# rodluger/starry_process

Measured on AMD Instinct MI355X. Metric: log_likelihood evals/sec (ydeg=15, K=1000), higher is better.
Workload: dtype f64

## Files before the change

### starry_process_amd/csrc/sp_cov.h

```cpp
#ifndef SP_COV_H
#define SP_COV_H

#include "sp_internal.h"

__device__ __forceinline__ int star_nobs(const sp_star &st, int K) {
  return (st.nobs > 0 && st.nobs < K) ? st.nobs : K;
}

__device__ __forceinline__ double temporal_factor(int kind, double ti, double tj,
                                                  double tau) {
#pragma clang fp contract(off)
  if (kind == SP_TEMPORAL_NONE) return 1.0;
  const double dt = fabs(ti - tj);
  if (kind == SP_TEMPORAL_MATERN32) {
    const double x = 1.7320508075688772 * dt / tau;
    return (1.0 + x) * exp(-x);
  }
  return exp(-(dt * dt) / (2.0 * tau));
}

__device__ __forceinline__ double temporal_dfactor_dtau(int kind, double ti, double tj,
                                                        double tau) {
  if (kind == SP_TEMPORAL_NONE) return 0.0;
  const double dt = fabs(ti - tj);
  if (kind == SP_TEMPORAL_MATERN32) {
    const double x = 1.7320508075688772 * dt / tau;
    return x * x / tau * exp(-x);
  }
  return (dt * dt) / (2.0 * tau * tau) * exp(-(dt * dt) / (2.0 * tau));
}

template <int CTRL>
__device__ __forceinline__ double dpp_move(double v) {
  const int lo = __builtin_amdgcn_mov_dpp(__double2loint(v), CTRL, 0xf, 0xf, true);
  const int hi = __builtin_amdgcn_mov_dpp(__double2hiint(v), CTRL, 0xf, 0xf, true);
  return __hiloint2double(hi, lo);
}
template <int N>
__device__ __forceinline__ void row16_sum(double (&x)[N]) {
#pragma unroll
  for (int k = 0; k < N; ++k) x[k] += dpp_move<0xB1>(x[k]);
#pragma unroll
  for (int k = 0; k < N; ++k) x[k] += dpp_move<0x4E>(x[k]);
#pragma unroll
  for (int k = 0; k < N; ++k) x[k] += dpp_move<0x141>(x[k]);
#pragma unroll
  for (int k = 0; k < N; ++k) x[k] += dpp_move<0x140>(x[k]);
}

typedef double dd2 __attribute__((ext_vector_type(2)));

struct SplineGen {
  const double *tab;
  int np2;
  double dx, inv_dx;
  int covpts;
  __device__ __forceinline__ double operator()(double thi, double thj) const {
#pragma clang fp contract(off)
    const double x = fabs(thi - thj);
    const double q = x * inv_dx;
    int idx = (int)q;
    double x0 = q - (double)idx;
    if (fabs(x0 - 0.5) > 0.5 - 1.0e-9) {
      idx = (int)floor(x / dx);
      x0 = q - (double)idx;
    }
    idx = idx > covpts ? covpts : idx;
    typedef const __attribute__((address_space(3))) dd2 *lds_dd2;
    const unsigned a1 = (unsigned)(size_t)(const __attribute__((address_space(3))) double *)tab + ((unsigned)idx << 4);
    const dd2 c01 = *(lds_dd2)(size_t)a1;
    const dd2 c23 = *(lds_dd2)(size_t)(a1 + 8u * (unsigned)np2);
    return __builtin_fma(x0, __builtin_fma(x0, __builtin_fma(x0, c23.y, c23.x), c01.y), c01.x);
  }
  template <int N>
  __device__ __forceinline__ void many(const double (&thi)[N], const double (&thj)[N], double (&out)[N]) const {
#pragma clang fp contract(off)
    double x0[N];
    int idx[N];
    bool odd = false;
#pragma unroll
    for (int e = 0; e < N; ++e) {
      const double q = fabs(thi[e] - thj[e]) * inv_dx;
      idx[e] = (int)q;
      x0[e] = q - (double)idx[e];
      odd |= fabs(x0[e] - 0.5) > 0.5 - 1.0e-9;
    }
    if (__builtin_expect(odd, 0)) {
#pragma unroll
      for (int e = 0; e < N; ++e)
        if (fabs(x0[e] - 0.5) > 0.5 - 1.0e-9) {
          const double x = fabs(thi[e] - thj[e]);
          idx[e] = (int)floor(x / dx);
          x0[e] = x * inv_dx - (double)idx[e];
        }
    }
    dd2 c01[N], c23[N];
    typedef const __attribute__((address_space(3))) dd2 *lds_dd2;
    const unsigned base = (unsigned)(size_t)(const __attribute__((address_space(3))) double *)tab;
    const unsigned off2 = 8u * (unsigned)np2;
#pragma unroll
    for (int e = 0; e < N; ++e) {
      const int k = idx[e] > covpts ? covpts : idx[e];
      const unsigned a1 = base + ((unsigned)k << 4);
      c01[e] = *(lds_dd2)(size_t)a1;
      c23[e] = *(lds_dd2)(size_t)(a1 + off2);
    }
#pragma unroll
    for (int e = 0; e < N; ++e)
      out[e] = __builtin_fma(x0[e], __builtin_fma(x0[e], __builtin_fma(x0[e], c23[e].y, c23[e].x), c01[e].y), c01[e].x);
  }
};


__device__ __forceinline__ void spline_table_to_lds(const double *__restrict__ src, double *stage, int np, int tid) {
  const int n2 = 2 * np;
  dd2 v[4];
#pragma unroll
  for (int c = 0; c < 4; ++c) {
    const int e = tid + 256 * c;
    v[c] = e < n2 ? *reinterpret_cast<const dd2 *>(src + 2 * e) : dd2{0.0, 0.0};
  }
#pragma unroll
  for (int c = 0; c < 4; ++c) {
    const int e = tid + 256 * c;
    if (e < n2) *reinterpret_cast<dd2 *>(stage + 2 * e) = v[c];
  }
  for (int e = tid + 1024; e < n2; e += 256)
    *reinterpret_cast<dd2 *>(stage + 2 * e) = *reinterpret_cast<const dd2 *>(src + 2 * e);
}


#ifndef SP_LAZY_BATCH
#define SP_LAZY_BATCH 8
#endif
template <int MA, typename V4>
__device__ __forceinline__ void lazy_cov_tiles(const LazyCov &z, int star, const int (&ri)[MA][4],
                                               const int (&cj)[4], V4 (&out)[MA][4], double *stage) {
  const sp_star st = z.stars[star];
  const int nobs = star_nobs(st, z.K), np = z.covpts + 4;
  const double *th = z.theta + (size_t)star * z.K, *tt = z.t + (size_t)star * z.K;
  const bool tk = z.temporal != SP_TEMPORAL_NONE;
#ifdef SP_LAZY_NO_SEP
  const bool sep = false;
#else
  const bool sep = z.temporal == SP_TEMPORAL_MATERN32 && z.inorder && z.inorder[star] != 0.0;
#endif
  double thi[MA][4], ti[MA][4], thj[4], tj[4];
#pragma unroll
  for (int k = 0; k < 4; ++k) {
    const bool oj = cj[k] < nobs;
    thj[k] = oj ? th[cj[k]] : 0.0;
    tj[k] = (oj && tk) ? tt[cj[k]] : 0.0;
#pragma unroll
    for (int m = 0; m < MA; ++m) {
      const bool oi = ri[m][k] < nobs;
      thi[m][k] = oi ? th[ri[m][k]] : 0.0;
      ti[m][k] = (oi && tk) ? tt[ri[m][k]] : 0.0;
    }
  }
  const int c0 = cj[0] & ~63;
  const double tb = sep ? tt[c0 < nobs ? c0 : nobs - 1] : 0.0;
  spline_table_to_lds(z.ptab + (size_t)star * 4 * np, stage, np, threadIdx.x);
  __syncthreads();
  SplineGen g{stage, 2 * np, 6.283185307179586 / z.covpts,
              1.0 / (6.283185307179586 / z.covpts), z.covpts};
  const double cm = sep ? 1.7320508075688772 / st.tau : 0.0;
  double fc[4] = {1.0, 1.0, 1.0, 1.0};
  bool fok[4] = {false, false, false, false};
  if (sep) {
#pragma unroll
    for (int n = 0; n < 4; ++n) {
      const double a = cm * (tj[n] - tb);
      fok[n] = a < 600.0 && a >= 0.0;
      fc[n] = exp(fok[n] ? a : 0.0);
    }
  }
#pragma unroll
  for (int m = 0; m < MA; ++m) {
    double er[4] = {1.0, 1.0, 1.0, 1.0};
    if (sep) {
#pragma unroll
      for (int r = 0; r < 4; ++r) er[r] = exp(-(cm * (ti[m][r] - tb)));
    }
#pragma unroll
    for (int n0 = 0; n0 < 4; n0 += SP_LAZY_BATCH / 4) {
      double a[SP_LAZY_BATCH], b[SP_LAZY_BATCH], v[SP_LAZY_BATCH];
#pragma unroll
      for (int e = 0; e < SP_LAZY_BATCH; ++e) {
        a[e] = thi[m][e & 3];
        b[e] = thj[n0 + (e >> 2)];
      }
      g.many<SP_LAZY_BATCH>(a, b, v);
#pragma unroll
      for (int e = 0; e < SP_LAZY_BATCH; ++e) {
        const int n = n0 + (e >> 2), r = e & 3;
        double w = 0.0;
        if (ri[m][r] < nobs && cj[n] < nobs) {
#pragma clang fp contract(off)
          if (sep && fok[n]) {
            const double x = cm * (ti[m][r] - tj[n]);
            w = v[e] * ((1.0 + x) * (er[r] * fc[n]));
          } else {
            w = v[e] * temporal_factor(z.temporal, ti[m][r], tj[n], st.tau);
          }
        }
        out[m][n][r] = w;
      }
    }
    if (z.rid) {
#pragma unroll
      for (int r = 0; r < 4; ++r) {
        const int mr = ri[m][r] - z.K;
        if (mr < 0 || mr >= z.nrid) continue;
        const double *src = z.rid + ((size_t)star * (z.nrid + 1) + mr) * z.K;
        double x[4];
#pragma unroll
        for (int n = 0; n < 4; ++n) x[n] = src[cj[n] < z.K ? cj[n] : z.K - 1];
#pragma unroll
        for (int n = 0; n < 4; ++n) out[m][n][r] = cj[n] < z.K ? x[n] : 0.0;
      }
    }
  }
  __syncthreads();
}

template <typename V4>
__device__ __forceinline__ void lazy_diag_block(const LazyCov &z, int star, const SplineGen &g, const sp_star &st,
                                                int nobs, const int (&ri)[4], int cj, V4 &out) {
  const double *th = z.theta + (size_t)star * z.K, *tt = z.t + (size_t)star * z.K;
  const double *rb = z.rid + (size_t)star * (z.nrid + 1) * z.K;
  const bool tk = z.temporal != SP_TEMPORAL_NONE;
  const int cc = cj < z.K ? cj : z.K - 1;
  const double thj = th[cc], tj = tk ? tt[cc] : 0.0;
  double thi[4], ti[4], dd[4], rv[4];
#pragma unroll
  for (int r = 0; r < 4; ++r) {
    const int rc = ri[r] < z.K ? ri[r] : z.K - 1;
    thi[r] = th[rc];
    ti[r] = tk ? tt[rc] : 0.0;
    dd[r] = rb[(size_t)z.nrid * z.K + rc];
    const int m = ri[r] - z.K;
    rv[r] = rb[(size_t)((m >= 0 && m < z.nrid) ? m : 0) * z.K + cc];
  }
#pragma unroll
  for (int r = 0; r < 4; ++r) {
    const int m = ri[r] - z.K;
    double v;
    if (ri[r] < nobs && cj < nobs) {
#pragma clang fp contract(off)
      v = g(thi[r], thj) * temporal_factor(z.temporal, ti[r], tj, st.tau);
      if (ri[r] == cj) v += dd[r];
    } else if (m >= 0 && m < z.nrid && cj < z.K) {
      v = rv[r];
    } else {
      v = ri[r] == cj ? 1.0 : 0.0;
    }
    out[r] = v;
  }
}

#ifndef SP_LAZY_ROW_BATCH
#define SP_LAZY_ROW_BATCH 0
#endif
template <int ROWB, typename V4>
__device__ __forceinline__ void lazy_cov_row(const LazyCov &z, int star, int ri, int c0, V4 (&out)[4],
                                             double *stage, int tid) {
  const sp_star st = z.stars[star];
  const int nobs = star_nobs(st, z.K), np = z.covpts + 4;
  const double *th = z.theta + (size_t)star * z.K;
  const bool oi = ri < nobs;
  const double thi = oi ? th[ri] : 0.0;
  double *s_thj = stage + 4 * np;
  {
    const double *src = z.ptab + (size_t)star * 4 * np;
    const int n2 = 2 * np, cbase = c0 & ~63;
    dd2 v[3];
#pragma unroll
    for (int c = 0; c < 3; ++c) {
      const int e = tid + 256 * c;
      v[c] = e < n2 ? *reinterpret_cast<const dd2 *>(src + 2 * e) : dd2{0.0, 0.0};
    }
    const double tj = (tid < 64 && cbase + tid < nobs) ? th[cbase + tid] : 0.0;
#pragma unroll
    for (int c = 0; c < 3; ++c) {
      const int e = tid + 256 * c;
      if (e < n2) *reinterpret_cast<dd2 *>(stage + 2 * e) = v[c];
    }
    for (int e = tid + 768; e < n2; e += 256)
      *reinterpret_cast<dd2 *>(stage + 2 * e) = *reinterpret_cast<const dd2 *>(src + 2 * e);
    if (tid < 64) s_thj[tid] = tj;
  }
  __syncthreads();
  SplineGen g{stage, 2 * np, 6.283185307179586 / z.covpts,
              1.0 / (6.283185307179586 / z.covpts), z.covpts};
  const int cl = c0 & 63;
  if constexpr (ROWB == 2) {
#pragma unroll
  for (int m = 0; m < 4; ++m) {
    V4 o;
#pragma unroll
    for (int half = 0; half < 2; ++half) {
      const dd2 tt = *reinterpret_cast<const dd2 *>(s_thj + cl + 16 * m + 2 * half);
      const double a[2] = {thi, thi}, b[2] = {tt.x, tt.y};
      double v[2];
      g.many<2>(a, b, v);
      o[2 * half] = (oi && c0 + 16 * m + 2 * half < nobs) ? v[0] : 0.0;
      o[2 * half + 1] = (oi && c0 + 16 * m + 2 * half + 1 < nobs) ? v[1] : 0.0;
      __builtin_amdgcn_sched_barrier(0);
    }
    out[m] = o;
  }
  } else if constexpr (ROWB == 0) {
#pragma unroll
  for (int m = 0; m < 4; ++m) {
    const dd2 t01 = *reinterpret_cast<const dd2 *>(s_thj + cl + 16 * m), t23 = *reinterpret_cast<const dd2 *>(s_thj + cl + 16 * m + 2);
    const double thj[4] = {t01.x, t01.y, t23.x, t23.y};
    V4 o;
#pragma unroll
    for (int r = 0; r < 4; ++r) o[r] = (oi && c0 + 16 * m + r < nobs) ? g(thi, thj[r]) : 0.0;
    out[m] = o;
  }
  } else {
#pragma unroll
  for (int m0 = 0; m0 < 4; m0 += ROWB / 4) {
    double a[ROWB], b[ROWB], v[ROWB];
#pragma unroll
    for (int h = 0; h < ROWB / 4; ++h) {
      const dd2 t01 = *reinterpret_cast<const dd2 *>(s_thj + cl + 16 * (m0 + h));
      const dd2 t23 = *reinterpret_cast<const dd2 *>(s_thj + cl + 16 * (m0 + h) + 2);
      a[4 * h] = a[4 * h + 1] = a[4 * h + 2] = a[4 * h + 3] = thi;
      b[4 * h] = t01.x;
      b[4 * h + 1] = t01.y;
      b[4 * h + 2] = t23.x;
      b[4 * h + 3] = t23.y;
    }
    g.many<ROWB>(a, b, v);
#pragma unroll
    for (int h = 0; h < ROWB / 4; ++h) {
      V4 o;
#pragma unroll
      for (int r = 0; r < 4; ++r) o[r] = (oi && c0 + 16 * (m0 + h) + r < nobs) ? v[4 * h + r] : 0.0;
      out[m0 + h] = o;
    }
    __builtin_amdgcn_sched_barrier(0);
  }
  }
  if (z.rid && !oi) {
    const int mr = ri - z.K;
    if (mr >= 0 && mr < z.nrid) {
      const double *src = z.rid + ((size_t)star * (z.nrid + 1) + mr) * z.K;
      double x[16];
#pragma unroll
      for (int e = 0; e < 16; ++e) {
        const int c = c0 + 16 * (e >> 2) + (e & 3);
        x[e] = src[c < z.K ? c : z.K - 1];
      }
#pragma unroll
      for (int m = 0; m < 4; ++m) {
        V4 o;
#pragma unroll
        for (int r = 0; r < 4; ++r) o[r] = c0 + 16 * m + r < z.K ? x[4 * m + r] : 0.0;
        out[m] = o;
      }
    }
  }
  __syncthreads();
}

#endif
```

### starry_process_amd/csrc/sp_gemm.hip

```cpp
#include <cstdlib>

#include <type_traits>

#include "sp_internal.h"
#include "sp_tile.h"
#include "sp_cov.h"
#include "sp_mm.h"
#include "sp_stage.h"
#include "sp_paneldiag.h"

typedef double d2 __attribute__((ext_vector_type(2)));

#define GT SP_GT

namespace {

__global__ __launch_bounds__(256) void gemm_nt_kernel(
    const double *A, long lda, long strideA, const double *__restrict__ B, long ldb, long strideB,
    double *C, long ldc, long strideC, int Mrows, int Nrows, int Kd, double alpha, int beta,
    int lower_only, int batch, int ntn, int ntiles, const int32_t *__restrict__ bsel, int nsel) {
  constexpr int BK = 32, LDW = BK + 1;
  __shared__ __attribute__((aligned(16))) double smem[2 * GT * LDW];
  double *sA = smem, *sB = smem + GT * LDW;
  int mtx, tile;
  if (!sp_xcd_decode(blockIdx.x, batch, ntiles, mtx, tile)) return;
  int ti, tj;
  if (lower_only) {
    ti = (int)((sqrt(8.0 * tile + 1.0) - 1.0) * 0.5);
    while (ti * (ti + 1) / 2 > tile) --ti;
    while ((ti + 1) * (ti + 2) / 2 <= tile) ++ti;
    tj = tile - ti * (ti + 1) / 2;
  } else {
    ti = tile / ntn;
    tj = tile % ntn;
  }
  const int row0 = ti * GT, col0 = tj * GT;
  const double *Ab = A + (size_t)mtx * strideA;
  int bm = mtx;
  if (bsel) {
    bm = bsel[mtx];
    if (bm < 0 || bm >= nsel) bm = 0;
  }
  const double *Bb = B + (size_t)bm * strideB;
  double *Cb = C + (size_t)mtx * strideC;
  const int lane = threadIdx.x & 63, wave = threadIdx.x >> 6;
  const int fr = lane & 15, fk = lane >> 4;
  d4 acc[4];
#pragma unroll
  for (int n = 0; n < 4; ++n) acc[n] = d4{0.0, 0.0, 0.0, 0.0};
  const bool full = row0 + GT <= Mrows && col0 + GT <= Nrows;
  if (beta) {
#pragma unroll
    for (int n = 0; n < 4; ++n)
#pragma unroll
      for (int r = 0; r < 4; ++r) {
        const int gi = row0 + 16 * wave + fk + 4 * r, gj = col0 + 16 * n + fr;
        if (full || (gi < Mrows && gj < Nrows)) acc[n][r] = Cb[(size_t)gi * ldc + gj];
      }
  }
  const bool vecA = ((lda & 1) == 0) && ((reinterpret_cast<uintptr_t>(Ab) & 15) == 0);
  const bool vecB = ((ldb & 1) == 0) && ((reinterpret_cast<uintptr_t>(Bb) & 15) == 0);
  PanelRegs<BK> ra, rb;
  if (Kd > 0) {
    stage_load<BK>(Ab, lda, row0, Mrows, 0, Kd, vecA, ra);
    stage_load<BK>(Bb, ldb, col0, Nrows, 0, Kd, vecB, rb);
  }
  for (int k0 = 0; k0 < Kd; k0 += BK) {
    stage_store<BK>(ra, alpha, sA);
    stage_store<BK>(rb, 1.0, sB);
    __syncthreads();
    if (k0 + BK < Kd) {
      stage_load<BK>(Ab, lda, row0, Mrows, k0 + BK, Kd, vecA, ra);
      stage_load<BK>(Bb, ldb, col0, Nrows, k0 + BK, Kd, vecB, rb);
    }
    const double *pa = sA + (16 * wave + fr) * LDW + fk;
    const double *pb = sB + fr * LDW + fk;
#pragma unroll
    for (int kk = 0; kk < BK; kk += 4) {
      const double a = pa[kk];
      acc[0] = __builtin_amdgcn_mfma_f64_16x16x4f64(a, pb[kk], acc[0], 0, 0, 0);
      acc[1] = __builtin_amdgcn_mfma_f64_16x16x4f64(a, pb[16 * LDW + kk], acc[1], 0, 0, 0);
      acc[2] = __builtin_amdgcn_mfma_f64_16x16x4f64(a, pb[32 * LDW + kk], acc[2], 0, 0, 0);
      acc[3] = __builtin_amdgcn_mfma_f64_16x16x4f64(a, pb[48 * LDW + kk], acc[3], 0, 0, 0);
    }
    __syncthreads();
  }
#pragma unroll
  for (int n = 0; n < 4; ++n)
#pragma unroll
    for (int r = 0; r < 4; ++r) {
      const int gi = row0 + 16 * wave + fk + 4 * r, gj = col0 + 16 * n + fr;
      if (full || (gi < Mrows && gj < Nrows)) Cb[(size_t)gi * ldc + gj] = acc[n][r];
    }
}

}

namespace {
#ifdef SP_MM_STAMPS
__device__ long long sp_mm_dbg[8 * 4096];
#endif
#ifndef SP_MM_WAVES
#define SP_MM_WAVES 1
#endif
#ifndef SP_MM_SYRK_NS
#define SP_MM_SYRK_NS 6
#endif
template <class Core, bool SGN, bool SEL = false>
__global__ __launch_bounds__(256, SP_MM_WAVES) void mm_nt_kernel(
    const double *__restrict__ A, long lda, long strideA, const double *__restrict__ B, long ldb,
    long strideB, double *__restrict__ C, long ldc, long strideC, int Kd, double alpha, int beta,
    int lower_only, int batch, int ntn, int ntiles, int skip00, LazyCov lz, DiagFuse df,
    const int32_t *__restrict__ bsel, int nsel) {
  constexpr int TM = Core::TM_, TN = Core::TN_;
  static_assert(Core::LDS_DOUBLES >= SP_DIAG_LDS_DOUBLES, "the tile-(0,0) workgroup factors a pivot block in this LDS");
  __shared__ __attribute__((aligned(16))) double lds[Core::LDS_DOUBLES];
#ifdef SP_MM_STAMPS
  const long long wall_begin = wall_clock64(), cyc_begin = __builtin_readcyclecounter();
#endif
  int mtx, tile;
  if (!sp_xcd_decode(blockIdx.x, batch, ntiles, mtx, tile)) return;
  int ti, tj;
  if (lower_only) {
    ti = (int)((sqrt(8.0 * tile + 1.0) - 1.0) * 0.5);
    while (ti * (ti + 1) / 2 > tile) --ti;
    while ((ti + 1) * (ti + 2) / 2 <= tile) ++ti;
    tj = tile - ti * (ti + 1) / 2;
  } else {
    ti = tile / ntn;
    tj = tile % ntn;
  }
  const int tj_limit = skip00 >> 8;
  int k_first = (skip00 & 2) ? ti * TM : 0;
  if (df.tri0 >= 0 && TM == 64) {
    const int r = 64 * (df.j + ti) - df.tri0, first = r > 0 ? r / 64 - df.s0 : 0;
    if (first > 0) k_first = 64 * first < Kd ? 64 * first : Kd;
  }
  if (tj_limit && tj >= tj_limit) return;
  if ((skip00 & 1) && lower_only && ti == 0 && tj == 0) {
    if (df.sys) {
      __builtin_amdgcn_s_setprio(3);
      panel_diag_item(df.sys + (size_t)mtx * df.stride, df.ld, df.j, df.nact,
                      df.img + (size_t)mtx * df.lts + sp_img_off(df.j),
                      df.info ? df.info + mtx : nullptr, lds, threadIdx.x);
    }
    return;
  }
  const double *Ab = A + (size_t)mtx * strideA + (size_t)ti * TM * lda;
  int bm = mtx;
  if constexpr (SEL) {
    bm = bsel[mtx];
    if (bm < 0 || bm >= nsel) bm = 0;
  }
  const double *Bb = B + (size_t)bm * strideB + (size_t)tj * TN * ldb;
  double *Cb = C + (size_t)mtx * strideC + (size_t)ti * TM * ldc + (size_t)tj * TN;
  Core mm;
  mm.init(Ab, lda, Bb, ldb);
  if constexpr (SGN && Core::MA == 1 && Core::NA == 4 && TM == 64 && TN == 64) {
    if ((skip00 & 4) && lower_only && ti == tj) {
      const bool dform = beta && lz.theta && (lz.dlazy & 2);
      const int lane = threadIdx.x & 63;
      sp_star dst{};
      int dnobs = 0;
      if (dform) {
        dst = lz.stars[mtx];
        dnobs = star_nobs(dst, lz.K);
        spline_table_to_lds(lz.ptab + (size_t)mtx * 4 * (lz.covpts + 4), lds, lz.covpts + 4, threadIdx.x);
        __syncthreads();
      }
      const SplineGen dg{lds, 2 * (lz.covpts + 4), 6.283185307179586 / lz.covpts, 1.0 / (6.283185307179586 / lz.covpts),
                         lz.covpts};
      if (!dform) mm.prologue(lds, k_first, Kd);
      auto run = [&](auto wtag) {
        constexpr int W = decltype(wtag)::value;
        using D = typename Core::template SymDeal<W>;
        mm_d4 a3[3];
#pragma unroll
        for (int b = 0; b < 3; ++b) {
          mm_d4 c = mm_d4{0.0, 0.0, 0.0, 0.0};
          if (b < D::NB && dform) {
            int ri[4];
#pragma unroll
            for (int r = 0; r < 4; ++r) ri[r] = 64 * (lz.tr0 + ti) + 16 * D::brow(b) + (lane >> 4) + 4 * r;
            lazy_diag_block(lz, mtx, dg, dst, dnobs, ri, 64 * (lz.tc0 + tj) + 16 * D::bcol(b) + (lane & 15), c);
          } else if (b < D::NB && beta) {
#pragma unroll
            for (int r = 0; r < 4; ++r)
              c[r] = Cb[(size_t)(16 * D::brow(b) + (lane >> 4) + 4 * r) * ldc + 16 * D::bcol(b) + (lane & 15)];
          }
          a3[b] = alpha < 0.0 ? -c : c;
        }
        if (dform) {
          __syncthreads();
          mm.prologue(lds, k_first, Kd);
        }
        mm.template sym_loop<W>(lds, k_first, Kd, a3);
#pragma unroll
        for (int b = 0; b < D::NB; ++b)
#pragma unroll
          for (int r = 0; r < 4; ++r)
            Cb[(size_t)(16 * D::brow(b) + (lane >> 4) + 4 * r) * ldc + 16 * D::bcol(b) + (lane & 15)] =
                alpha < 0.0 ? -a3[b][r] : a3[b][r];
      };
      switch (threadIdx.x >> 6) {
        case 0: run(std::integral_constant<int, 0>{}); break;
        case 1: run(std::integral_constant<int, 1>{}); break;
        case 2: run(std::integral_constant<int, 2>{}); break;
        default: run(std::integral_constant<int, 3>{}); break;
      }
      return;
    }
  }
  mm_d4 acc[Core::MA][Core::NA], cin[SGN ? 1 : Core::MA][SGN ? 1 : Core::NA];
  constexpr bool CAN_LAZY = Core::MA == 1 && Core::NA == 4 && TM == 64 && TN == 64;
  const bool lazy = CAN_LAZY && beta && lz.theta && lz.tr0 + ti > lz.tc0 + tj && lz.tc0 + tj > 0 &&
                    lz.tr0 + ti < lz.nfull;
  mm_d4 cz1[1][4];
  mm_d4 (&cz)[4] = cz1[0];
  if (!lazy) mm.prologue(lds, k_first, Kd);
  if (lazy) {
    int ri[1][4], cj[4];
#pragma unroll
    for (int k = 0; k < 4; ++k) {
      ri[0][k] = 64 * (lz.tr0 + ti) + mm.acc_row(0, k);
      cj[k] = 64 * (lz.tc0 + tj) + mm.acc_col(k < Core::NA ? k : 0);
    }
    lazy_cov_tiles<1>(lz, mtx, ri, cj, cz1, lds);
    mm.prologue(lds, k_first, Kd);
  }
#pragma unroll
  for (int m = 0; m < Core::MA; ++m)
#pragma unroll
    for (int n = 0; n < Core::NA; ++n) {
      mm_d4 c = mm_d4{0.0, 0.0, 0.0, 0.0};
      if (lazy) {
        c = cz[n & 3];
      } else if (beta) {
#pragma unroll
        for (int r = 0; r < 4; ++r) c[r] = Cb[(size_t)mm.acc_row(m, r) * ldc + mm.acc_col(n)];
      }
      if (SGN) {
        acc[m][n] = alpha < 0.0 ? -c : c;
      } else {
        acc[m][n] = mm_d4{0.0, 0.0, 0.0, 0.0};
        cin[m][n] = c;
      }
    }
#ifdef SP_MM_STAMPS
  const long long cyc_loop = __builtin_readcyclecounter();
#endif
  mm.loop(lds, k_first, Kd, acc);
#ifdef SP_MM_STAMPS
  const long long cyc_store = __builtin_readcyclecounter();
#endif
#pragma unroll
  for (int m = 0; m < Core::MA; ++m)
#pragma unroll
    for (int n = 0; n < Core::NA; ++n)
#pragma unroll
      for (int r = 0; r < 4; ++r) {
        double v;
        if (SGN)
          v = alpha < 0.0 ? -acc[m][n][r] : acc[m][n][r];
        else
          v = fma(alpha, acc[m][n][r], cin[m][n][r]);
        Cb[(size_t)mm.acc_row(m, r) * ldc + mm.acc_col(n)] = v;
      }
#ifdef SP_MM_STAMPS
  if (threadIdx.x == 0 && lower_only && df.sys && blockIdx.x < 4096) {
    long long *o = sp_mm_dbg + 8 * blockIdx.x;
    o[0] = (long long)mtx * 4096 + tile; o[1] = lazy; o[2] = wall_begin; o[3] = wall_clock64();
    o[4] = cyc_loop - cyc_begin; o[5] = cyc_store - cyc_loop; o[6] = __builtin_readcyclecounter() - cyc_store;
    o[7] = ((__builtin_amdgcn_s_getreg(20 | (0 << 6) | (31 << 11)) & 15u) << 8) | ((__builtin_amdgcn_s_getreg(4 | (0 << 6) | (31 << 11)) >> 8) & 255u);
  }
#endif
}


using Syrk128Core = MM2<128, 64, 8, 4, 4>;
#ifndef SP_SYRK128_WGS
#define SP_SYRK128_WGS 1
#endif
__global__ __launch_bounds__(256, SP_SYRK128_WGS) void syrk128_kernel(const double *__restrict__ X, long ld, long stride,
                                                      double *__restrict__ T, int Kd, int batch, int nb, int ntiles,
                                                      LazyCov lz, DiagFuse df) {
  using Core = Syrk128Core;
  static_assert(Core::LDS_DOUBLES >= SP_DIAG_LDS_DOUBLES, "the last workgroup of a star factors a pivot block in this LDS");
  static_assert(Core::MA == 2 && Core::NA == 4, "a wavefront = 32 rows of one block row");
  __shared__ __attribute__((aligned(16))) double lds[Core::LDS_DOUBLES];
  int mtx, tile;
  if (!sp_xcd_decode(blockIdx.x, batch, ntiles, mtx, tile)) return;
  if (tile == 0) {
    if (df.sys) {
      __builtin_amdgcn_s_setprio(3);
      panel_diag_item(df.sys + (size_t)mtx * df.stride, df.ld, df.j, df.nact,
                      df.img + (size_t)mtx * df.lts + sp_img_off(df.j), df.info ? df.info + mtx : nullptr, lds, threadIdx.x);
    }
    return;
  }
  tile -= 1;
  const int o = nb & 1;
  int I = (int)((sqrt((double)((o + 1) * (o + 1) + 4 * tile)) - (o + 1)) * 0.5);
  while (I * I + I * (o + 1) > tile) --I;
  while ((I + 1) * (I + 1) + (I + 1) * (o + 1) <= tile) ++I;
  const int J = tile - (I * I + I * (o + 1)), R0 = o + 2 * I;
  const double *Xb = X + (size_t)mtx * stride;
  const double *Ab = Xb + (size_t)R0 * 64 * ld, *Bb = Xb + (size_t)J * 64 * ld;
  double *Cb = T + (size_t)mtx * stride + (size_t)R0 * 64 * ld + (size_t)J * 64;
  Core mm;
  mm.init(Ab, ld, Bb, ld);
  const int R = R0 + (mm.acc_row(0, 0) >> 6);
  const bool want = R >= J && !(R == 0 && J == 0);
  const auto is_lazy = [&](int Rb) {
    return lz.theta && lz.tr0 + Rb > lz.tc0 + J && lz.tc0 + J > 0 && lz.tr0 + Rb < lz.nfull;
  };
  const bool any_lazy = is_lazy(R0) || is_lazy(R0 + 1), my_lazy = is_lazy(R);
  mm_d4 acc[Core::MA][Core::NA];
  if (any_lazy) {
    int ri[Core::MA][4], cj[4];
#pragma unroll
    for (int k = 0; k < 4; ++k) {
      cj[k] = 64 * (lz.tc0 + J) + mm.acc_col(k);
#pragma unroll
      for (int m = 0; m < Core::MA; ++m) ri[m][k] = 64 * (lz.tr0 + R0) + mm.acc_row(m, k);
    }
    lazy_cov_tiles<Core::MA>(lz, mtx, ri, cj, acc, lds);
  }
  mm.prologue(lds, 0, Kd);
#pragma unroll
  for (int m = 0; m < Core::MA; ++m)
#pragma unroll
    for (int n = 0; n < Core::NA; ++n) {
      mm_d4 c = mm_d4{0.0, 0.0, 0.0, 0.0};
      if (any_lazy && my_lazy) {
        c = acc[m][n];
      } else if (want) {
#pragma unroll
        for (int r = 0; r < 4; ++r) c[r] = Cb[(size_t)mm.acc_row(m, r) * ld + mm.acc_col(n)];
      }
      acc[m][n] = -c;
    }
  mm.loop(lds, 0, Kd, acc);
  if (!want) return;
#pragma unroll
  for (int m = 0; m < Core::MA; ++m)
#pragma unroll
    for (int n = 0; n < Core::NA; ++n)
#pragma unroll
      for (int r = 0; r < 4; ++r) Cb[(size_t)mm.acc_row(m, r) * ld + mm.acc_col(n)] = -acc[m][n][r];
}

template <class Core>
int mm_launch(const double *A, long lda, long strideA, const double *B, long ldb, long strideB,
              double *C, long ldc, long strideC, int Mrows, int Nrows, int Kd, double alpha, int beta,
              int lower_only, int batch, hipStream_t st, int skip00, const LazyCov *lazy = nullptr,
              const DiagFuse *dfp = nullptr, const int32_t *bsel = nullptr, int nsel = 0) {
  const LazyCov lz = lazy ? *lazy : LazyCov{};
  const DiagFuse df = dfp ? *dfp : DiagFuse{nullptr, 0, 0, 0, 0, nullptr, 0, nullptr, -1, 0};
  const int ntm = Mrows / Core::TM_, ntn = Nrows / Core::TN_;
  const int ntiles = lower_only ? ntm * (ntm + 1) / 2 : ntm * ntn;
  const long nblk = sp_xcd_grid(batch, ntiles);
  if (nblk > 0x7fffffffL) return SP_ERR_INVALID;
  if (bsel) {
    if (alpha != 1.0 || lazy || dfp) return SP_ERR_INVALID;
    hipLaunchKernelGGL((mm_nt_kernel<Core, true, true>), dim3((unsigned)nblk), dim3(256), 0, st,
                       A, lda, strideA, B, ldb, strideB, C, ldc, strideC, Kd, alpha, beta, lower_only,
                       batch, ntn, ntiles, skip00, lz, df, bsel, nsel);
  } else if (alpha == 1.0 || alpha == -1.0)
    hipLaunchKernelGGL((mm_nt_kernel<Core, true>), dim3((unsigned)nblk), dim3(256), 0, st,
                       A, lda, strideA, B, ldb, strideB, C, ldc, strideC, Kd, alpha, beta, lower_only,
                       batch, ntn, ntiles, skip00, lz, df, (const int32_t *)nullptr, 0);
  else
    hipLaunchKernelGGL((mm_nt_kernel<Core, false>), dim3((unsigned)nblk), dim3(256), 0, st,
                       A, lda, strideA, B, ldb, strideB, C, ldc, strideC, Kd, alpha, beta, lower_only,
                       batch, ntn, ntiles, skip00, lz, df, (const int32_t *)nullptr, 0);
  SP_LAUNCH_CHECK();
  return SP_OK;
}
}

#ifdef SP_MM_STAMPS
extern "C" int sp_debug_mm_stamps(long long *out, int n) {
  return (int)hipMemcpyFromSymbol(out, HIP_SYMBOL(sp_mm_dbg), sizeof(long long) * n);
}
#endif

static int launch_gemm(const double *A, long lda, long strideA, const double *B, long ldb,
                       long strideB, double *C, long ldc, long strideC, int Mrows, int Nrows,
                       int Kd, double alpha, int beta, int lower_only, int batch, hipStream_t st,
                       int skip00 = 0, const LazyCov *lazy = nullptr, const int32_t *bsel = nullptr, int nsel = 0) {
  if (bsel && (nsel < 1 || skip00 || (lazy && lazy->theta))) return SP_ERR_INVALID;
  if (Mrows <= 0 || Nrows <= 0 || batch <= 0) return SP_OK;
  if (Kd < 0) return SP_ERR_INVALID;
  const int ntm = (Mrows + GT - 1) / GT, ntn = (Nrows + GT - 1) / GT;
  if (lower_only && ntm != ntn) return SP_ERR_INVALID;
  const int ntiles = lower_only ? ntm * (ntm + 1) / 2 : ntm * ntn;
  const long nblk = sp_xcd_grid(batch, ntiles);
  if (nblk > 0x7fffffffL) return SP_ERR_INVALID;
  const bool fast = (Mrows % GT) == 0 && (Nrows % GT) == 0 && (Kd % 32) == 0 && Kd > 0 &&
                    ((lda | ldb) & 1) == 0 && (strideA & 1) == 0 && (strideB & 1) == 0 &&
                    ((reinterpret_cast<uintptr_t>(A) | reinterpret_cast<uintptr_t>(B)) & 15) == 0;
  if (lazy && lazy->theta) {
    if (!fast) return SP_ERR_INVALID;
    return mm_launch<MM2<64, 64, 8, 6, 4>>(A, lda, strideA, B, ldb, strideB, C, ldc, strideC, Mrows, Nrows,
                                           Kd, alpha, beta, lower_only, batch, st, skip00, lazy);
  }
  if (fast) {
#ifdef SP_MM_TILE_PROBE
    static const int probe = getenv("SP_MM_TILE") ? atoi(getenv("SP_MM_TILE")) : 0;
    if (!bsel && !lower_only && probe == 1 && (Mrows % 128) == 0)
      return mm_launch<MM2<128, 64, 8, 4, 4>>(A, lda, strideA, B, ldb, strideB, C, ldc, strideC, Mrows, Nrows, Kd, alpha,
                                              beta, lower_only, batch, st, skip00);
    if (!bsel && !lower_only && probe == 2 && (Mrows % 128) == 0)
      return mm_launch<MM2<128, 64, 8, 5, 4>>(A, lda, strideA, B, ldb, strideB, C, ldc, strideC, Mrows, Nrows, Kd, alpha,
                                              beta, lower_only, batch, st, skip00);
    if (!bsel && !lower_only && probe == 3 && (Mrows % 128) == 0)
      return mm_launch<MM2<128, 64, 16, 3, 4>>(A, lda, strideA, B, ldb, strideB, C, ldc, strideC, Mrows, Nrows, Kd, alpha,
                                               beta, lower_only, batch, st, skip00);
    if (!bsel && !lower_only && probe == 4)
      return mm_launch<MM2<64, 64, 8, 6, 4>>(A, lda, strideA, B, ldb, strideB, C, ldc, strideC, Mrows, Nrows, Kd, alpha,
                                             beta, lower_only, batch, st, skip00);
#endif
    if (!lower_only && (Mrows % 128) == 0 && (Nrows % 128) == 0)
      return mm_launch<MM2<128, 128, 8, 4, 2>>(A, lda, strideA, B, ldb, strideB, C, ldc, strideC, Mrows,
                                               Nrows, Kd, alpha, beta, lower_only, batch, st, skip00, nullptr, nullptr,
// ... 43 lines not shown
```

### starry_process_amd/csrc/sp_panel.hip

```cpp
#include "sp_internal.h"
#include "sp_tile.h"
#include "sp_cov.h"
#include "sp_stage.h"
#include "sp_paneldiag.h"
#include "sp_reduce.h"
#include <atomic>

#ifdef SP_PANEL_TRACE
__device__ long long g_p2trace[64 * 3 * 16];
__device__ long long g_p2chain[16 * 64 * 4];
__device__ int g_p2cu[16 * 1024];
__device__ long long g_p2wg[16 * 1024 * 2];
struct P2WgStamp {
  int j, on;
  __device__ P2WgStamp(int j_, bool on_) : j(j_), on(on_ && j_ < 16 && blockIdx.x < 1024 && threadIdx.x == 0) {
    if (on) g_p2wg[(j * 1024 + blockIdx.x) * 2] = wall_clock64();
  }
  __device__ ~P2WgStamp() {
    if (on) g_p2wg[(j * 1024 + blockIdx.x) * 2 + 1] = wall_clock64();
  }
};
#define P2_CHAIN(k, v)                                                                          \
  do {                                                                                          \
    if (tid == 0 && a.j < 16 && mtx < 64) g_p2chain[((a.j * 64) + mtx) * 4 + (k)] = (v);        \
  } while (0)
#define P2_STAMP(role, k)                                                                       \
  do {                                                                                          \
    if (mtx == 0 && tid == 0 && a.j < 64 && (role) >= 0) g_p2trace[(a.j * 3 + (role)) * 16 + (k)] = wall_clock64(); \
  } while (0)
#else
#define P2_STAMP(role, k) do { } while (0)
#define P2_CHAIN(k, v) do { } while (0)
#endif

#ifndef P_WGS
#define P_WGS 3
#endif

namespace {

constexpr int PK = 32;
constexpr int PLDW = PK + 1;
constexpr int XLD = 66;
__device__ __forceinline__ constexpr int sx_col(int nb, int fk) { return 32 * (fk & 1) + 8 * nb + 4 * (fk >> 1); }
#ifndef P_PAIRS
#define P_PAIRS 1
#endif
constexpr int P_LDS = P_PAIRS ? 3 * 64 * PLDW
                              : SP_DIAG_LDS_DOUBLES;
static_assert(P_LDS >= SP_DIAG_LDS_DOUBLES && P_LDS >= 64 * XLD && P_LDS >= SP_IMG_DOUBLES,
              "one LDS region, four tenants in turn");

enum { P_DITEMS = 1,
       P_TITEMS = 2,
       P_TAILD = 4,
       P_LOOKAHEAD = 8,
       P_FIRSTLA = 16 };

struct PanelArgs {
  double *sys;
  long ld, stride;
  int S, ntile;
  int j, s0;
  int nact;
  int next_nact;
  int last;
  int mode;
  int pair;
  int lay;
  int seq;
  int tri0;
  double *img;
  long lts;
  int32_t *info;
  LazyCov lz;
  SpReduceArgs red;
};

typedef double pd4 __attribute__((ext_vector_type(4)));

__device__ __forceinline__ long long cu_key() {
  const unsigned hw = __builtin_amdgcn_s_getreg(4 | (8 << 6) | (7 << 11));
  const unsigned xcc = __builtin_amdgcn_s_getreg(20 | (0 << 6) | (3 << 11)) & 7u;
  return (long long)(xcc * 256 + hw);
}

__host__ __device__ __forceinline__ int panel_titems(int ntile, int j, int pair) {
  const int n = ntile - j - 1;
  return n <= 0 ? 0 : (pair ? 1 + n / 2 : n);
}

template <int NR, bool LAZY, bool RED, bool CHAIN>
__device__ __forceinline__ void panel_tile_item(const PanelArgs &a, double *M, int mtx, int i0, int cb,
                                                int kb0, int kb1, bool la, bool may_lazy,
                                                double *img_star, double *smem, int tid) {
  const int lane = tid & 63, wave = tid >> 6, fr = lane & 15, fk = lane >> 4;
  const long ld = a.ld;
#ifdef P_NO_PRODUCT
  const int Kd = 0 * (kb1 - kb0);
#else
  const int Kd = 64 * (kb1 - kb0);
#endif
  const double *img = img_star + sp_img_off(a.j);
  const bool chain = CHAIN && NR == 1 && !la && i0 == a.j + 1 && (a.mode & P_TAILD);
#ifdef SP_PANEL_TRACE
  const int role = i0 == a.j + 1 ? 1 : (i0 + NR == a.ntile ? 2 : -1);
#endif
  P2_STAMP(role, 0);
  if (NR == 1 && !la && i0 == a.j + 1) P2_CHAIN(0, wall_clock64());
#ifndef P_NO_CHAIN_PRIO
  if (chain) __builtin_amdgcn_s_setprio(3);
#endif
  double *Ct = M + (size_t)(64 * i0) * ld + 64 * cb;
  const double *Ab = M + (size_t)(64 * i0) * ld + 64 * kb0;
  const double *Bb = M + (size_t)(64 * cb) * ld + 64 * kb0;
  double *sA = smem, *sB = smem + NR * 64 * PLDW;

  pd4 g[NR][4];
  double *crow = Ct + (size_t)(16 * wave + fr) * ld + 4 * fk;
#ifndef P_IMG_PREFETCH
#define P_IMG_PREFETCH 1
#endif
  PanelRegs<PK> ra[NR], rb;
  const bool any_lazy = LAZY && may_lazy && a.lz.theta && (cb > 0 || a.lz.c0lazy) && i0 < a.lz.nfull;
  auto first_loads = [&]() {
#pragma unroll
    for (int h = 0; h < NR; ++h) stage_load_fast<PK>(Ab, ld, 64 * h, 0, ra[h], tid);
    stage_load_fast<PK>(Bb, ld, 0, 0, rb, tid);
  };
  if (Kd > 0 && !any_lazy) first_loads();
#pragma unroll
  for (int h = 0; h < NR; ++h) {
    const bool lazy = LAZY && may_lazy && a.lz.theta && (cb > 0 || a.lz.c0lazy) && i0 + h < a.lz.nfull;
    if (!lazy) {
#pragma unroll
      for (int m = 0; m < 4; ++m) {
        const d2v lo = *reinterpret_cast<const d2v *>(crow + (size_t)(64 * h) * ld + 16 * m);
        const d2v hi = *reinterpret_cast<const d2v *>(crow + (size_t)(64 * h) * ld + 16 * m + 2);
        g[h][m] = pd4{lo.x, lo.y, hi.x, hi.y};
      }
    } else {
#ifdef P_NO_LAZYEVAL
#pragma unroll
      for (int m = 0; m < 4; ++m) g[h][m] = pd4{0.0, 0.0, 0.0, 1.0e-3 * (m + fk)};
#else
      lazy_cov_row<(NR == 1 ? SP_LAZY_ROW_BATCH : 0)>(a.lz, mtx, 64 * (i0 + h) + 16 * wave + fr, 64 * cb + 4 * fk, g[h], smem, tid);
#endif
    }
  }
  if (Kd > 0 && any_lazy) first_loads();
  P2_STAMP(role, 1);

  d2v im[5];
  auto image_loads = [&](bool now = false) {
    if (la || (!(P_IMG_PREFETCH && NR == 1) && !now)) return;
#pragma unroll
    for (int c = 0; c < 5; ++c) im[c] = *reinterpret_cast<const d2v *>(img + 2 * (tid + 256 * c));
  };
  if (Kd == 0) image_loads(true);

  {
    const int pfr = sp_pi16(fr);
    auto mfma_slice = [&]() {
      const double *pa = sB + pfr * PLDW + fk;
      const double *pb = sA + (16 * wave + fr) * PLDW + fk;
#pragma clang loop unroll_count(NR == 2 ? 2 : 8)
      for (int kk = 0; kk < PK; kk += 4) {
        const double a0 = pa[kk], a1 = pa[16 * PLDW + kk], a2 = pa[32 * PLDW + kk], a3 = pa[48 * PLDW + kk];
#pragma unroll
        for (int h = 0; h < NR; ++h) {
          const double b = pb[h * 64 * PLDW + kk];
          g[h][0] = __builtin_amdgcn_mfma_f64_16x16x4f64(a0, b, g[h][0], 0, 0, 0);
          g[h][1] = __builtin_amdgcn_mfma_f64_16x16x4f64(a1, b, g[h][1], 0, 0, 0);
          g[h][2] = __builtin_amdgcn_mfma_f64_16x16x4f64(a2, b, g[h][2], 0, 0, 0);
          g[h][3] = __builtin_amdgcn_mfma_f64_16x16x4f64(a3, b, g[h][3], 0, 0, 0);
        }
      }
    };
    int k0 = 0;
    for (; k0 + PK < Kd; k0 += PK) {
#pragma unroll
      for (int h = 0; h < NR; ++h) stage_store<PK>(ra[h], -1.0, sA + h * 64 * PLDW, tid);
      stage_store<PK>(rb, 1.0, sB, tid);
      __syncthreads();
#pragma unroll
      for (int h = 0; h < NR; ++h) stage_load_fast<PK>(Ab, ld, 64 * h, k0 + PK, ra[h], tid);
      stage_load_fast<PK>(Bb, ld, 0, k0 + PK, rb, tid);
      mfma_slice();
      __syncthreads();
    }
    if (k0 < Kd) {
#pragma unroll
      for (int h = 0; h < NR; ++h) stage_store<PK>(ra[h], -1.0, sA + h * 64 * PLDW, tid);
      stage_store<PK>(rb, 1.0, sB, tid);
      __syncthreads();
      image_loads();
      mfma_slice();
      __syncthreads();
    }
  }

  P2_STAMP(role, 2);
  if (la) {
#pragma unroll
    for (int h = 0; h < NR; ++h)
#pragma unroll
      for (int m = 0; m < 4; ++m) {
        double *dst = crow + (size_t)(64 * h) * ld + 16 * m;
        *reinterpret_cast<d2v *>(dst) = d2v{g[h][m][0], g[h][m][1]};
        *reinterpret_cast<d2v *>(dst + 2) = d2v{g[h][m][2], g[h][m][3]};
      }
    return;
  }
  P2_STAMP(role, 3);
  if (!(P_IMG_PREFETCH && NR == 1)) image_loads(true);
#pragma unroll
  for (int c = 0; c < 5; ++c) *reinterpret_cast<d2v *>(smem + 2 * (tid + 256 * c)) = im[c];
  __syncthreads();
  pd4 dacp[4];
#ifndef P_DAC_PREFETCH
#define P_DAC_PREFETCH 1
#endif
  if (P_DAC_PREFETCH && NR == 1 && i0 <= a.last) {
    const double *Dt0 = M + (size_t)(64 * i0) * ld + 64 * i0;
#pragma unroll
    for (int m = 0; m < 4; ++m)
      if (m <= wave) {
#pragma unroll
        for (int r = 0; r < 4; ++r) dacp[m][r] = Dt0[(size_t)(16 * wave + fk + 4 * r) * ld + 16 * m + fr];
      }
  }
  pd4 y[NR][4];
  {
    const double *fimg = smem + 2 * lane;
#pragma unroll
    for (int h = 0; h < NR; ++h) {
#pragma unroll
      for (int nb = 3; nb >= 0; --nb) {
        pd4 acc = pd4{0.0, 0.0, 0.0, 0.0};
#pragma unroll
        for (int kb = 0; kb <= nb; ++kb) {
          const double *f = fimg + sp_img_block(nb, kb) * 256;
          const d2v lo = *reinterpret_cast<const d2v *>(f);
          const d2v hi = *reinterpret_cast<const d2v *>(f + 128);
          acc = __builtin_amdgcn_mfma_f64_16x16x4f64(lo.x, g[h][kb][0], acc, 0, 0, 0);
          acc = __builtin_amdgcn_mfma_f64_16x16x4f64(lo.y, g[h][kb][1], acc, 0, 0, 0);
          acc = __builtin_amdgcn_mfma_f64_16x16x4f64(hi.x, g[h][kb][2], acc, 0, 0, 0);
          acc = __builtin_amdgcn_mfma_f64_16x16x4f64(hi.y, g[h][kb][3], acc, 0, 0, 0);
        }
        y[h][nb] = acc;
      }
      if (h == 0) P2_STAMP(role, 4);
#pragma unroll
      for (int nb = 0; nb < 4; ++nb) {
        double *dst = crow + (size_t)(64 * h) * ld + 16 * nb;
        *reinterpret_cast<d2v *>(dst) = d2v{y[h][nb][0], y[h][nb][1]};
        *reinterpret_cast<d2v *>(dst + 2) = d2v{y[h][nb][2], y[h][nb][3]};
      }
    }
  }
  P2_STAMP(role, 5);
#ifdef P_NO_EAGER
  return;
#endif
#pragma unroll
  for (int h = 0; h < NR; ++h) {
    const int i = i0 + h;
    if (i > a.last) break;
    double *sX = smem;
      __syncthreads();
#pragma unroll
    for (int nb = 0; nb < 4; ++nb) {
      double *dst = sX + (16 * wave + fr) * XLD + sx_col(nb, fk);
      *reinterpret_cast<d2v *>(dst) = d2v{y[h][nb][0], y[h][nb][1]};
      *reinterpret_cast<d2v *>(dst + 2) = d2v{y[h][nb][2], y[h][nb][3]};
    }
    double *Dt = M + (size_t)(64 * i) * ld + 64 * i;
    pd4 dac[4];
#pragma unroll
    for (int m = 0; m < 4; ++m) {
      if (P_DAC_PREFETCH && NR == 1 && h == 0) {
        dac[m] = dacp[m];
      } else if (m <= wave) {
#pragma unroll
        for (int r = 0; r < 4; ++r) dac[m][r] = Dt[(size_t)(16 * wave + fk + 4 * r) * ld + 16 * m + fr];
      }
    }
    __syncthreads();
#pragma unroll
    for (int nb = 0; nb < 4; ++nb) {
#pragma unroll
      for (int m = 0; m < 4; ++m) {
        if (m > wave) continue;
        const double *f = sX + (16 * m + fr) * XLD + sx_col(nb, fk);
        const d2v lo = *reinterpret_cast<const d2v *>(f);
        const d2v hi = *reinterpret_cast<const d2v *>(f + 2);
        dac[m] = __builtin_amdgcn_mfma_f64_16x16x4f64(-y[h][nb][0], lo.x, dac[m], 0, 0, 0);
        dac[m] = __builtin_amdgcn_mfma_f64_16x16x4f64(-y[h][nb][1], lo.y, dac[m], 0, 0, 0);
        dac[m] = __builtin_amdgcn_mfma_f64_16x16x4f64(-y[h][nb][2], hi.x, dac[m], 0, 0, 0);
        dac[m] = __builtin_amdgcn_mfma_f64_16x16x4f64(-y[h][nb][3], hi.y, dac[m], 0, 0, 0);
      }
    }
    if (!(chain && a.next_nact == 64)) {
// ... 254 lines not shown
```

Before: 107,500.

## Hoist lazy covariance global loads ahead of spline table staging and barriers

Splits spline table staging into separate load and store phases. The theta/t and diagonal-block global loads are issued before the LDS store and barrier, so their latency overlaps the table fetch. Bounds checks that depended on nobs become clamps to K-1, so loads no longer wait on the star record, and nobs/sep are computed after the loads. It also adds optional cycle stamps and an early-slice panel option, which is off by default. Clamped loads may fetch unused values, which are still masked later.

Result: no change. 107,600 (median of 6 runs) (+0.1%).

```diff
diff --git a/starry_process_amd/csrc/sp_cov.h b/starry_process_amd/csrc/sp_cov.h
--- a/starry_process_amd/csrc/sp_cov.h
+++ b/starry_process_amd/csrc/sp_cov.h
@@ -112,14 +112,17 @@
 };
 
 
-__device__ __forceinline__ void spline_table_to_lds(const double *__restrict__ src, double *stage, int np, int tid) {
+__device__ __forceinline__ void spline_table_load(const double *__restrict__ src, int np, int tid, dd2 (&v)[4]) {
   const int n2 = 2 * np;
-  dd2 v[4];
 #pragma unroll
   for (int c = 0; c < 4; ++c) {
     const int e = tid + 256 * c;
     v[c] = e < n2 ? *reinterpret_cast<const dd2 *>(src + 2 * e) : dd2{0.0, 0.0};
   }
+}
+__device__ __forceinline__ void spline_table_store(const double *__restrict__ src, double *stage, int np, int tid,
+                                                   const dd2 (&v)[4]) {
+  const int n2 = 2 * np;
 #pragma unroll
   for (int c = 0; c < 4; ++c) {
     const int e = tid + 256 * c;
@@ -128,40 +131,56 @@
   for (int e = tid + 1024; e < n2; e += 256)
     *reinterpret_cast<dd2 *>(stage + 2 * e) = *reinterpret_cast<const dd2 *>(src + 2 * e);
 }
+__device__ __forceinline__ void spline_table_to_lds(const double *__restrict__ src, double *stage, int np, int tid) {
+  dd2 v[4];
+  spline_table_load(src, np, tid, v);
+  spline_table_store(src, stage, np, tid, v);
+}
 
 
 #ifndef SP_LAZY_BATCH
 #define SP_LAZY_BATCH 8
 #endif
+__device__ __forceinline__ double lazy_load_at(const double *base, unsigned byte_offset) {
+  return *reinterpret_cast<const double *>(reinterpret_cast<const char *>(base) + byte_offset);
+}
 template <int MA, typename V4>
 __device__ __forceinline__ void lazy_cov_tiles(const LazyCov &z, int star, const int (&ri)[MA][4],
-                                               const int (&cj)[4], V4 (&out)[MA][4], double *stage) {
+                                               const int (&cj)[4], V4 (&out)[MA][4], double *stage,
+                                               long long *cyc = nullptr) {
   const sp_star st = z.stars[star];
-  const int nobs = star_nobs(st, z.K), np = z.covpts + 4;
+  const int np = z.covpts + 4, kl = z.K - 1;
   const double *th = z.theta + (size_t)star * z.K, *tt = z.t + (size_t)star * z.K;
   const bool tk = z.temporal != SP_TEMPORAL_NONE;
 #ifdef SP_LAZY_NO_SEP
-  const bool sep = false;
+  const bool maysep = false;
 #else
-  const bool sep = z.temporal == SP_TEMPORAL_MATERN32 && z.inorder && z.inorder[star] != 0.0;
+  const bool maysep = z.temporal == SP_TEMPORAL_MATERN32 && z.inorder;
 #endif
+  const double ord = *(maysep ? z.inorder + star : th);
   double thi[MA][4], ti[MA][4], thj[4], tj[4];
 #pragma unroll
   for (int k = 0; k < 4; ++k) {
-    const bool oj = cj[k] < nobs;
-    thj[k] = oj ? th[cj[k]] : 0.0;
-    tj[k] = (oj && tk) ? tt[cj[k]] : 0.0;
+    const unsigned cc = 8u * (unsigned)(cj[k] < kl ? cj[k] : kl);
+    thj[k] = lazy_load_at(th, cc);
+    tj[k] = tk ? lazy_load_at(tt, cc) : 0.0;
 #pragma unroll
     for (int m = 0; m < MA; ++m) {
-      const bool oi = ri[m][k] < nobs;
-      thi[m][k] = oi ? th[ri[m][k]] : 0.0;
-      ti[m][k] = (oi && tk) ? tt[ri[m][k]] : 0.0;
+      const unsigned rc = 8u * (unsigned)(ri[m][k] < kl ? ri[m][k] : kl);
+      thi[m][k] = lazy_load_at(th, rc);
+      ti[m][k] = tk ? lazy_load_at(tt, rc) : 0.0;
     }
   }
   const int c0 = cj[0] & ~63;
-  const double tb = sep ? tt[c0 < nobs ? c0 : nobs - 1] : 0.0;
-  spline_table_to_lds(z.ptab + (size_t)star * 4 * np, stage, np, threadIdx.x);
+  const double tb = maysep ? tt[c0 < kl ? c0 : kl] : 0.0;
+  dd2 tv[4];
+  spline_table_load(z.ptab + (size_t)star * 4 * np, np, threadIdx.x, tv);
+  if (cyc) cyc[0] = __builtin_readcyclecounter();
+  spline_table_store(z.ptab + (size_t)star * 4 * np, stage, np, threadIdx.x, tv);
+  const int nobs = star_nobs(st, z.K);
+  const bool sep = maysep && ord != 0.0;
   __syncthreads();
+  if (cyc) cyc[1] = __builtin_readcyclecounter();
   SplineGen g{stage, 2 * np, 6.283185307179586 / z.covpts,
               1.0 / (6.283185307179586 / z.covpts), z.covpts};
   const double cm = sep ? 1.7320508075688772 / st.tau : 0.0;
@@ -221,37 +240,44 @@
       }
     }
   }
+  if (cyc) cyc[2] = __builtin_readcyclecounter();
   __syncthreads();
-}
-
-template <typename V4>
-__device__ __forceinline__ void lazy_diag_block(const LazyCov &z, int star, const SplineGen &g, const sp_star &st,
-                                                int nobs, const int (&ri)[4], int cj, V4 &out) {
+  if (cyc) cyc[3] = __builtin_readcyclecounter();
+}
+
+struct LazyDiagLoads {
+  double thj, tj, thi[4], ti[4], dd[4], rv[4];
+};
+__device__ __forceinline__ void lazy_diag_load(const LazyCov &z, int star, const int (&ri)[4], int cj, LazyDiagLoads &l) {
   const double *th = z.theta + (size_t)star * z.K, *tt = z.t + (size_t)star * z.K;
   const double *rb = z.rid + (size_t)star * (z.nrid + 1) * z.K;
   const bool tk = z.temporal != SP_TEMPORAL_NONE;
   const int cc = cj < z.K ? cj : z.K - 1;
-  const double thj = th[cc], tj = tk ? tt[cc] : 0.0;
-  double thi[4], ti[4], dd[4], rv[4];
+  l.thj = th[cc];
+  l.tj = tk ? tt[cc] : 0.0;
 #pragma unroll
   for (int r = 0; r < 4; ++r) {
     const int rc = ri[r] < z.K ? ri[r] : z.K - 1;
-    thi[r] = th[rc];
-    ti[r] = tk ? tt[rc] : 0.0;
-    dd[r] = rb[(size_t)z.nrid * z.K + rc];
+    l.thi[r] = th[rc];
+    l.ti[r] = tk ? tt[rc] : 0.0;
+    l.dd[r] = rb[(size_t)z.nrid * z.K + rc];
     const int m = ri[r] - z.K;
-    rv[r] = rb[(size_t)((m >= 0 && m < z.nrid) ? m : 0) * z.K + cc];
-  }
+    l.rv[r] = rb[(size_t)((m >= 0 && m < z.nrid) ? m : 0) * z.K + cc];
+  }
+}
+template <typename V4>
+__device__ __forceinline__ void lazy_diag_block(const LazyCov &z, const SplineGen &g, const sp_star &st, int nobs,
+                                                const int (&ri)[4], int cj, const LazyDiagLoads &l, V4 &out) {
 #pragma unroll
   for (int r = 0; r < 4; ++r) {
     const int m = ri[r] - z.K;
     double v;
     if (ri[r] < nobs && cj < nobs) {
 #pragma clang fp contract(off)
-      v = g(thi[r], thj) * temporal_factor(z.temporal, ti[r], tj, st.tau);
-      if (ri[r] == cj) v += dd[r];
+      v = g(l.thi[r], l.thj) * temporal_factor(z.temporal, l.ti[r], l.tj, st.tau);
+      if (ri[r] == cj) v += l.dd[r];
     } else if (m >= 0 && m < z.nrid && cj < z.K) {
-      v = rv[r];
+      v = l.rv[r];
     } else {
       v = ri[r] == cj ? 1.0 : 0.0;
     }
@@ -266,10 +292,9 @@
 __device__ __forceinline__ void lazy_cov_row(const LazyCov &z, int star, int ri, int c0, V4 (&out)[4],
                                              double *stage, int tid) {
   const sp_star st = z.stars[star];
-  const int nobs = star_nobs(st, z.K), np = z.covpts + 4;
+  const int np = z.covpts + 4, kl = z.K - 1;
   const double *th = z.theta + (size_t)star * z.K;
-  const bool oi = ri < nobs;
-  const double thi = oi ? th[ri] : 0.0;
+  const double thi = th[ri < kl ? ri : kl];
   double *s_thj = stage + 4 * np;
   {
     const double *src = z.ptab + (size_t)star * 4 * np;
@@ -280,7 +305,7 @@
       const int e = tid + 256 * c;
       v[c] = e < n2 ? *reinterpret_cast<const dd2 *>(src + 2 * e) : dd2{0.0, 0.0};
     }
-    const double tj = (tid < 64 && cbase + tid < nobs) ? th[cbase + tid] : 0.0;
+    const double tj = tid < 64 ? th[cbase + tid < kl ? cbase + tid : kl] : 0.0;
 #pragma unroll
     for (int c = 0; c < 3; ++c) {
       const int e = tid + 256 * c;
@@ -290,6 +315,8 @@
       *reinterpret_cast<dd2 *>(stage + 2 * e) = *reinterpret_cast<const dd2 *>(src + 2 * e);
     if (tid < 64) s_thj[tid] = tj;
   }
+  const int nobs = star_nobs(st, z.K);
+  const bool oi = ri < nobs;
   __syncthreads();
   SplineGen g{stage, 2 * np, 6.283185307179586 / z.covpts,
               1.0 / (6.283185307179586 / z.covpts), z.covpts};
@@ -345,9 +372,9 @@
     __builtin_amdgcn_sched_barrier(0);
   }
   }
-  if (z.rid && !oi) {
+  if (z.rid && ri >= z.K) {
     const int mr = ri - z.K;
-    if (mr >= 0 && mr < z.nrid) {
+    if (mr < z.nrid) {
       const double *src = z.rid + ((size_t)star * (z.nrid + 1) + mr) * z.K;
       double x[16];
 #pragma unroll
diff --git a/starry_process_amd/csrc/sp_gemm.hip b/starry_process_amd/csrc/sp_gemm.hip
--- a/starry_process_amd/csrc/sp_gemm.hip
+++ b/starry_process_amd/csrc/sp_gemm.hip
@@ -98,7 +98,7 @@
 
 namespace {
 #ifdef SP_MM_STAMPS
-__device__ long long sp_mm_dbg[8 * 4096];
+__device__ long long sp_mm_dbg[12 * 4096];
 #endif
 #ifndef SP_MM_WAVES
 #define SP_MM_WAVES 1
@@ -117,6 +117,7 @@
   __shared__ __attribute__((aligned(16))) double lds[Core::LDS_DOUBLES];
 #ifdef SP_MM_STAMPS
   const long long wall_begin = wall_clock64(), cyc_begin = __builtin_readcyclecounter();
+  long long cyc_form[4] = {0, 0, 0, 0};
 #endif
   int mtx, tile;
   if (!sp_xcd_decode(blockIdx.x, batch, ntiles, mtx, tile)) return;
@@ -160,39 +161,46 @@
     if ((skip00 & 4) && lower_only && ti == tj) {
       const bool dform = beta && lz.theta && (lz.dlazy & 2);
       const int lane = threadIdx.x & 63;
-      sp_star dst{};
-      int dnobs = 0;
-      if (dform) {
-        dst = lz.stars[mtx];
-        dnobs = star_nobs(dst, lz.K);
-        spline_table_to_lds(lz.ptab + (size_t)mtx * 4 * (lz.covpts + 4), lds, lz.covpts + 4, threadIdx.x);
-        __syncthreads();
-      }
-      const SplineGen dg{lds, 2 * (lz.covpts + 4), 6.283185307179586 / lz.covpts, 1.0 / (6.283185307179586 / lz.covpts),
-                         lz.covpts};
+      const int dnp = lz.covpts + 4;
+      const SplineGen dg{lds, 2 * dnp, 6.283185307179586 / lz.covpts, 1.0 / (6.283185307179586 / lz.covpts), lz.covpts};
       if (!dform) mm.prologue(lds, k_first, Kd);
       auto run = [&](auto wtag) {
         constexpr int W = decltype(wtag)::value;
         using D = typename Core::template SymDeal<W>;
         mm_d4 a3[3];
-#pragma unroll
-        for (int b = 0; b < 3; ++b) {
-          mm_d4 c = mm_d4{0.0, 0.0, 0.0, 0.0};
-          if (b < D::NB && dform) {
-            int ri[4];
-#pragma unroll
-            for (int r = 0; r < 4; ++r) ri[r] = 64 * (lz.tr0 + ti) + 16 * D::brow(b) + (lane >> 4) + 4 * r;
-            lazy_diag_block(lz, mtx, dg, dst, dnobs, ri, 64 * (lz.tc0 + tj) + 16 * D::bcol(b) + (lane & 15), c);
-          } else if (b < D::NB && beta) {
-#pragma unroll
-            for (int r = 0; r < 4; ++r)
-              c[r] = Cb[(size_t)(16 * D::brow(b) + (lane >> 4) + 4 * r) * ldc + 16 * D::bcol(b) + (lane & 15)];
+        if (dform) {
+          const sp_star dst = lz.stars[mtx];
+          int ri[D::NB][4], cj[D::NB];
+          LazyDiagLoads dl[D::NB];
+#pragma unroll
+          for (int b = 0; b < D::NB; ++b) {
+#pragma unroll
+            for (int r = 0; r < 4; ++r) ri[b][r] = 64 * (lz.tr0 + ti) + 16 * D::brow(b) + (lane >> 4) + 4 * r;
+            cj[b] = 64 * (lz.tc0 + tj) + 16 * D::bcol(b) + (lane & 15);
+            lazy_diag_load(lz, mtx, ri[b], cj[b], dl[b]);
           }
-          a3[b] = alpha < 0.0 ? -c : c;
-        }
-        if (dform) {
+          spline_table_to_lds(lz.ptab + (size_t)mtx * 4 * dnp, lds, dnp, threadIdx.x);
+          const int dnobs = star_nobs(dst, lz.K);
+          __syncthreads();
+#pragma unroll
+          for (int b = 0; b < 3; ++b) {
+            mm_d4 c = mm_d4{0.0, 0.0, 0.0, 0.0};
+            if (b < D::NB) lazy_diag_block(lz, dg, dst, dnobs, ri[b % D::NB], cj[b % D::NB], dl[b % D::NB], c);
+            a3[b] = alpha < 0.0 ? -c : c;
+          }
           __syncthreads();
           mm.prologue(lds, k_first, Kd);
+        } else {
+#pragma unroll
+          for (int b = 0; b < 3; ++b) {
+            mm_d4 c = mm_d4{0.0, 0.0, 0.0, 0.0};
+            if (b < D::NB && beta) {
+#pragma unroll
+              for (int r = 0; r < 4; ++r)
+                c[r] = Cb[(size_t)(16 * D::brow(b) + (lane >> 4) + 4 * r) * ldc + 16 * D::bcol(b) + (lane & 15)];
+            }
+            a3[b] = alpha < 0.0 ? -c : c;
+          }
         }
         mm.template sym_loop<W>(lds, k_first, Kd, a3);
 #pragma unroll
@@ -225,7 +233,11 @@
       ri[0][k] = 64 * (lz.tr0 + ti) + mm.acc_row(0, k);
       cj[k] = 64 * (lz.tc0 + tj) + mm.acc_col(k < Core::NA ? k : 0);
     }
+#ifdef SP_MM_STAMPS
+    lazy_cov_tiles<1>(lz, mtx, ri, cj, cz1, lds, cyc_form);
+#else
     lazy_cov_tiles<1>(lz, mtx, ri, cj, cz1, lds);
+#endif
     mm.prologue(lds, k_first, Kd);
   }
 #pragma unroll
@@ -271,6 +283,7 @@
     long long *o = sp_mm_dbg + 8 * blockIdx.x;
     o[0] = (long long)mtx * 4096 + tile; o[1] = lazy; o[2] = wall_begin; o[3] = wall_clock64();
     o[4] = cyc_loop - cyc_begin; o[5] = cyc_store - cyc_loop; o[6] = __builtin_readcyclecounter() - cyc_store;
+    for (int k = 0; k < 4; ++k) sp_mm_dbg[8 * 4096 + 4 * blockIdx.x + k] = cyc_form[k] ? cyc_form[k] - cyc_begin : 0;
     o[7] = ((__builtin_amdgcn_s_getreg(20 | (0 << 6) | (31 << 11)) & 15u) << 8) | ((__builtin_amdgcn_s_getreg(4 | (0 << 6) | (31 << 11)) >> 8) & 255u);
   }
 #endif
diff --git a/starry_process_amd/csrc/sp_panel.hip b/starry_process_amd/csrc/sp_panel.hip
--- a/starry_process_amd/csrc/sp_panel.hip
+++ b/starry_process_amd/csrc/sp_panel.hip
@@ -35,6 +35,9 @@
 
 #ifndef P_WGS
 #define P_WGS 3
+#endif
+#ifndef SP_PANEL_EARLY_SLICES
+#define SP_PANEL_EARLY_SLICES 0
 #endif
 
 namespace {
@@ -128,7 +131,8 @@
     for (int h = 0; h < NR; ++h) stage_load_fast<PK>(Ab, ld, 64 * h, 0, ra[h], tid);
     stage_load_fast<PK>(Bb, ld, 0, 0, rb, tid);
   };
-  if (Kd > 0 && !any_lazy) first_loads();
+  constexpr bool early_slices = SP_PANEL_EARLY_SLICES && NR == 1;
+  if (Kd > 0 && (!any_lazy || early_slices)) first_loads();
 #pragma unroll
   for (int h = 0; h < NR; ++h) {
     const bool lazy = LAZY && may_lazy && a.lz.theta && (cb > 0 || a.lz.c0lazy) && i0 + h < a.lz.nfull;
@@ -148,7 +152,7 @@
 #endif
     }
   }
-  if (Kd > 0 && any_lazy) first_loads();
+  if (Kd > 0 && any_lazy && !early_slices) first_loads();
   P2_STAMP(role, 1);
 
   d2v im[5];
```
